# semchan/DCT_Pruning

Measured on AMD Instinct MI355X. Metric: feature-map DCT+score throughput, higher is better.
Workload: dtype f32; 1 GPU; resnet_50 hooked feature maps (49 tensors, 22720 maps/sample: 56x56 x1344, 28x28 x3200, 14x14 x9472, 7x7 x8704), batch 256, limit=steps; global_batch=256, launch_mode=one launch per tile shape, units_rank0=49

## Files before the change

dct_pruning_amd/csrc/dct_codelets.hpp:

```cpp
#pragma once

#include <utility>

#if defined(__HIPCC__)
#define DCTS_HD __host__ __device__ __forceinline__
#else
#define DCTS_HD inline __attribute__((always_inline))
#endif

namespace dcts {

constexpr double kPi = 3.14159265358979323846264338327950288;

constexpr double cx_sin_taylor(double x) {
  const double x2 = x * x;
  double term = x, sum = x;
  for (int i = 1; i <= 12; ++i) {
    term *= -x2 / double((2 * i) * (2 * i + 1));
    sum += term;
  }
  return sum;
}
constexpr double cx_cos_taylor(double x) {
  const double x2 = x * x;
  double term = 1.0, sum = 1.0;
  for (int i = 1; i <= 12; ++i) {
    term *= -x2 / double((2 * i - 1) * (2 * i));
    sum += term;
  }
  return sum;
}
constexpr double cospi_frac(long long p, long long q) {
  long long r = p % (2 * q);
  if (r < 0) r += 2 * q;
  if (r > q) r = 2 * q - r;
  double sign = 1.0;
  if (2 * r > q) {
    r = q - r;
    sign = -1.0;
  }
  if (4 * r > q) {
    return sign * cx_sin_taylor(kPi * double(q - 2 * r) / double(2 * q));
  }
  return sign * cx_cos_taylor(kPi * double(r) / double(q));
}
constexpr double sinpi_frac(long long p, long long q) {
  return cospi_frac(q - 2 * p, 2 * q);
}

template <class F, int... I>
DCTS_HD void static_for_impl(F&& f, std::integer_sequence<int, I...>) {
  (f(std::integral_constant<int, I>{}), ...);
}
template <int N, class F>
DCTS_HD void static_for(F&& f) {
  static_for_impl(static_cast<F&&>(f), std::make_integer_sequence<int, N>{});
}

#define DCTS_LAMBDA_INLINE __attribute__((always_inline))

typedef float f2 __attribute__((vector_size(8)));

template <class T>
struct is_pair {
  static constexpr bool value = false;
};
template <>
struct is_pair<f2> {
  static constexpr bool value = true;
};

template <int N>
struct Dct2;
template <int M>
struct Dct4;

template <int M>
struct Dct4 {
  template <class T>
  static DCTS_HD void run(const T (&v)[M], T (&X)[M]) {
    if constexpr (M == 1) {
      constexpr float c = float(cospi_frac(1, 4));
      X[0] = v[0] * c;
    } else if constexpr (M % 2 == 0) {
      constexpr int H = M / 2;
#ifdef DCTS_PAIRS
      if constexpr (!is_pair<T>::value) {
        f2 ab[H];
        static_for<H>([&](auto i) DCTS_LAMBDA_INLINE {
          constexpr int n = decltype(i)::value;
          constexpr float c = float(cospi_frac(2 * n + 1, 4 * M));
          constexpr float s = float(sinpi_frac(2 * n + 1, 4 * M));
          constexpr float sg = (n % 2 == 0) ? 1.0f : -1.0f;
          const f2 p = {v[n], v[M - 1 - n]}, q = {v[M - 1 - n], v[n]};
          const f2 cc = {c, sg * c}, ss = {s, -sg * s};
          ab[n] = p * cc + q * ss;
        });
        f2 AB[H];
        Dct2<H>::run(ab, AB);
        X[0] = AB[0][0];
        X[M - 1] = -AB[0][1];
        static_for<H - 1>([&](auto i) DCTS_LAMBDA_INLINE {
          constexpr int j = decltype(i)::value + 1;
          X[2 * j] = AB[j][0] + AB[H - j][1];
          X[2 * j - 1] = AB[j][0] - AB[H - j][1];
        });
        return;
      }
#endif
      T a[H], b[H];
      static_for<H>([&](auto i) DCTS_LAMBDA_INLINE {
        constexpr int n = decltype(i)::value;
        constexpr float c = float(cospi_frac(2 * n + 1, 4 * M));
        constexpr float s = float(sinpi_frac(2 * n + 1, 4 * M));
        constexpr float sg = (n % 2 == 0) ? 1.0f : -1.0f;
        a[n] = v[n] * c + v[M - 1 - n] * s;
        b[n] = v[M - 1 - n] * (sg * c) - v[n] * (sg * s);
      });
      T A[H], B[H];
      Dct2<H>::run(a, A);
      Dct2<H>::run(b, B);
      X[0] = A[0];
      X[M - 1] = -B[0];
      static_for<H - 1>([&](auto i) DCTS_LAMBDA_INLINE {
        constexpr int j = decltype(i)::value + 1;
        X[2 * j] = A[j] + B[H - j];
        X[2 * j - 1] = A[j] - B[H - j];
      });
    } else {
      static_for<M>([&](auto ik) DCTS_LAMBDA_INLINE {
        constexpr int k = decltype(ik)::value;
        T acc{};
        static_for<M>([&](auto in) DCTS_LAMBDA_INLINE {
          constexpr int n = decltype(in)::value;
          constexpr float c = float(cospi_frac((2 * n + 1) * (2 * k + 1), 4 * M));
          if constexpr (n == 0)
            acc = v[0] * c;
          else
            acc += v[n] * c;
        });
        X[k] = acc;
      });
    }
  }
};

template <int N>
struct Dct2 {
  template <class T>
  static DCTS_HD void run(const T (&x)[N], T (&X)[N]) {
    if constexpr (N == 1) {
      X[0] = x[0];
    } else if constexpr (N % 2 == 0) {
      constexpr int H = N / 2;
      T u[H], v[H];
      static_for<H>([&](auto i) DCTS_LAMBDA_INLINE {
        constexpr int n = decltype(i)::value;
        u[n] = x[n] + x[N - 1 - n];
        v[n] = x[n] - x[N - 1 - n];
      });
      T E[H], O[H];
      Dct2<H>::run(u, E);
      Dct4<H>::run(v, O);
      static_for<H>([&](auto i) DCTS_LAMBDA_INLINE {
        constexpr int k = decltype(i)::value;
        X[2 * k] = E[k];
        X[2 * k + 1] = O[k];
      });
    } else {
      constexpr int m = (N - 1) / 2;
      T u[m], v[m];
      static_for<m>([&](auto i) DCTS_LAMBDA_INLINE {
        constexpr int n = decltype(i)::value;
        u[n] = x[n] + x[N - 1 - n];
        v[n] = x[n] - x[N - 1 - n];
      });
      const T mid = x[m];
      static_for<N>([&](auto ik) DCTS_LAMBDA_INLINE {
        constexpr int k = decltype(ik)::value;
        if constexpr (k == 0) {
          T acc = mid;
          static_for<m>([&](auto in) DCTS_LAMBDA_INLINE { acc += u[decltype(in)::value]; });
          X[0] = acc;
        } else if constexpr (k % 2 == 0) {
          T acc = ((k / 2) % 2 == 0) ? mid : -mid;
          static_for<m>([&](auto in) DCTS_LAMBDA_INLINE {
            constexpr int n = decltype(in)::value;
            constexpr float c = float(cospi_frac((2 * n + 1) * k, 2 * N));
            acc += u[n] * c;
          });
          X[k] = acc;
        } else {
          T acc{};
          static_for<m>([&](auto in) DCTS_LAMBDA_INLINE {
            constexpr int n = decltype(in)::value;
            constexpr float c = float(cospi_frac((2 * n + 1) * k, 2 * N));
            if constexpr (n == 0)
              acc = v[0] * c;
            else
              acc += v[n] * c;
          });
          X[k] = acc;
        }
      });
    }
  }
};

constexpr double cx_sqrt(double a) {
  if (a <= 0.0) return 0.0;
  double x = a > 1.0 ? a : 1.0;
  for (int i = 0; i < 200; ++i) x = 0.5 * (x + a / x);
  return x;
}
template <int N>
constexpr float ortho_scale(int k) {
  return float(k == 0 ? cx_sqrt(1.0 / double(N)) : cx_sqrt(2.0 / double(N)));
}
constexpr float kInvSqrt2 = float(0.70710678118654752440084436210484903928);

}
```

Before: 3722 Mmaps/s.

## Use symmetric index-mapping factorization for odd-length DCT-IV codelets

Replaces the direct O(M^2) matrix evaluation of odd-length DCT-IV (except M=3) with a factorization that permutes inputs and outputs via modular index maps. It forms sum and difference pairs and splits the output into cosine and sine halves sharing common terms. This roughly halves the multiplies for sizes like 7, which the 7x7 and 14x14 maps reach through the DCT-II recursion. It adds compile-time index logic and changes float rounding order, and any sign-pairing mistake would produce wrong coefficients.

```diff
diff --git a/dct_pruning_amd/csrc/dct_codelets.hpp b/dct_pruning_amd/csrc/dct_codelets.hpp
--- a/dct_pruning_amd/csrc/dct_codelets.hpp
+++ b/dct_pruning_amd/csrc/dct_codelets.hpp
@@ -47,6 +47,24 @@
 constexpr double sinpi_frac(long long p, long long q) {
   return cospi_frac(q - 2 * p, 2 * q);
 }
+
+constexpr int inv_mod(int a, int q) {
+  for (int x = 1; x < q; ++x)
+    if ((a * x) % q == 1) return x;
+  return 0;
+}
+constexpr int odd_index(int j, int M) {
+  for (int n = 0; n < M; ++n)
+    if ((2 * n + 1) % M == j) return n;
+  return -1;
+}
+constexpr int out_index(int kp, int M, int w) {
+  for (int k = 0; k < M; ++k)
+    if ((w * (2 * k + 1)) % M == kp) return k;
+  return -1;
+}
+constexpr int chi_c(int t) { return (t % 8 == 1 || t % 8 == 7) ? 1 : -1; }
+constexpr int chi_s(int t) { return (t % 8 == 1 || t % 8 == 3) ? 1 : -1; }
 
 template <class F, int... I>
 DCTS_HD void static_for_impl(F&& f, std::integer_sequence<int, I...>) {
@@ -127,7 +145,7 @@
         X[2 * j] = A[j] + B[H - j];
         X[2 * j - 1] = A[j] - B[H - j];
       });
-    } else {
+    } else if constexpr (M == 3) {
       static_for<M>([&](auto ik) DCTS_LAMBDA_INLINE {
         constexpr int k = decltype(ik)::value;
         T acc{};
@@ -140,6 +158,85 @@
             acc += v[n] * c;
         });
         X[k] = acc;
+      });
+    } else {
+      constexpr int m = (M - 1) / 2;
+      constexpr int u = inv_mod(M % 8, 8), w = inv_mod(8 % M, M);
+      constexpr double r = cospi_frac(1, 4);
+      T d[m];
+      static_for<m>([&](auto ij) DCTS_LAMBDA_INLINE {
+        constexpr int j = decltype(ij)::value + 1;
+        constexpr int n1 = odd_index(j, M), n2 = odd_index(M - j, M);
+        if constexpr (chi_s(2 * n1 + 1) == chi_s(2 * n2 + 1))
+          d[j - 1] = v[n1] - v[n2];
+        else
+          d[j - 1] = v[n1] + v[n2];
+      });
+      T Sg[m];
+      static_for<m>([&](auto ik) DCTS_LAMBDA_INLINE {
+        constexpr int kp = decltype(ik)::value + 1;
+        constexpr int kA = out_index(kp, M, w), kB = out_index(M - kp, M, w);
+        constexpr int abA = chi_c(2 * kA + 1) * chi_c(u) * chi_s(2 * kA + 1) * chi_s(u);
+        constexpr int abB = chi_c(2 * kB + 1) * chi_c(u) * chi_s(2 * kB + 1) * chi_s(u);
+        static_assert(abA == abB, "odd DCT-IV: sign pairing");
+        static_for<m>([&](auto ij) DCTS_LAMBDA_INLINE {
+          constexpr int j = decltype(ij)::value + 1;
+          constexpr int a1 = 2 * odd_index(j, M) + 1;
+          constexpr float ss = float(abA * chi_s(a1) * r * sinpi_frac(2 * j * kp, M));
+          if constexpr (j == 1)
+            Sg[kp - 1] = d[0] * ss;
+          else
+            Sg[kp - 1] += d[j - 1] * ss;
+        });
+      });
+      T s[m];
+      static_for<m>([&](auto ij) DCTS_LAMBDA_INLINE {
+        constexpr int j = decltype(ij)::value + 1;
+        constexpr int n1 = odd_index(j, M), n2 = odd_index(M - j, M);
+        if constexpr (chi_c(2 * n1 + 1) == chi_c(2 * n2 + 1))
+          s[j - 1] = v[n1] + v[n2];
+        else
+          s[j - 1] = v[n1] - v[n2];
+      });
+      constexpr float r0 = float(chi_c(M) * r);
+      const T t0 = v[m] * r0;
+      {
+        constexpr int k = odd_index(0, M);
+        constexpr int al = chi_c(2 * k + 1) * chi_c(u);
+        constexpr int g1 = chi_c(2 * odd_index(1, M) + 1);
+        T sum = s[0];
+        static_for<m - 1>([&](auto ij) DCTS_LAMBDA_INLINE {
+          constexpr int j = decltype(ij)::value + 2;
+          if constexpr (chi_c(2 * odd_index(j, M) + 1) == g1)
+            sum += s[j - 1];
+          else
+            sum -= s[j - 1];
+        });
+        constexpr float rg = float(g1 * r);
+        if constexpr (al > 0)
+          X[k] = sum * rg + t0;
+        else
+          X[k] = sum * (-rg) - t0;
+      }
+      static_for<m>([&](auto ik) DCTS_LAMBDA_INLINE {
+        constexpr int kp = decltype(ik)::value + 1;
+        constexpr int kA = out_index(kp, M, w), kB = out_index(M - kp, M, w);
+        constexpr int alA = chi_c(2 * kA + 1) * chi_c(u), alB = chi_c(2 * kB + 1) * chi_c(u);
+        T C = t0;
+        static_for<m>([&](auto ij) DCTS_LAMBDA_INLINE {
+          constexpr int j = decltype(ij)::value + 1;
+          constexpr int a1 = 2 * odd_index(j, M) + 1;
+          constexpr float cc = float(chi_c(a1) * r * cospi_frac(2 * j * kp, M));
+          C += s[j - 1] * cc;
+        });
+        if constexpr (alA > 0)
+          X[kA] = C - Sg[kp - 1];
+        else
+          X[kA] = Sg[kp - 1] - C;
+        if constexpr (alB > 0)
+          X[kB] = C + Sg[kp - 1];
+        else
+          X[kB] = -C - Sg[kp - 1];
       });
     }
   }
```

Result: faster. 3768 Mmaps/s (median of 6 runs) (+1.2%).
